# innate2adaptive/decombinator

Hardware: NVIDIA B200
Metric: decombined_reads_per_sec (higher is better)
Workload: dtype u32

## Files before the change

decombinator_b200/csrc/dcb_tables.h:

```cpp
#ifndef DCB_TABLES_H
#define DCB_TABLES_H

#include <stdint.h>

#define DCB_MAX_TAG_LEN 32
#define DCB_MAX_TAGS 255
#define DCB_MAX_READ_LEN 4096
#define DCB_HASH_EMPTY 0xFFFFFFFFu

struct DcbKw {
    uint32_t bits_lo, bits_hi;
    uint8_t len;
    uint8_t first_tag;
    uint8_t n_tags;
    uint8_t tags_off;
    uint32_t pad;
};

struct DcbKwSet {
    int32_t n_kw;
    int32_t kq;
    int32_t bitmap_off;
    int32_t hash_off;
    int32_t hash_mask;
    int32_t kw_off;
    int32_t taglist_off;
    int32_t min_len, max_len;
    int32_t set_id;
};

#define DCB_TAG_WORDS 12
struct DcbTag {
    uint32_t bits_lo, bits_hi;
    uint32_t mask_lo, mask_hi;
    uint32_t edge_lo, edge_hi;
    int16_t jump;
    int16_t region_len;
    uint8_t len;
    uint8_t edge_ok;
    uint8_t next_same_prefix;
    uint8_t pad8;
    int32_t region_off;
    uint32_t pad[3];
};

struct DcbGene {
    int32_t n_tags, split, is_v;
    int32_t tag_off;
    DcbKwSet full, half1, half2;
    int32_t lmin;
    int32_t n_words;
};

struct DcbSeedIndex {
    int32_t q, stride;
    int32_t max_off;
    int32_t wlead;
    int32_t lmin;
    int32_t wbits;
    uint32_t bmul;
    int32_t k, span;
    int32_t ck_off;
    uint32_t c1, c2;
    int32_t cshift;
    int32_t tk_off;
    uint32_t t1;
    int32_t tshift;
    int32_t utag_off;
    int32_t n_v, n_tags;
    int32_t chain_off;
    int32_t head_words;
    int32_t bloom_off;
    int32_t n_words;
    int32_t legacy_words;
    int32_t qq, qstride;
    int32_t fbits;
    uint32_t fmul;
    uint32_t m1, m2;
    int32_t b1, b2;
    int32_t qtab_off;
    int32_t qtab_words;
    int32_t bfilter_off;
    int32_t tq_off, tq_bits;
    uint32_t ta, tb;
    int32_t qwlead;
};
#define DCB_TQ_MORE (1u << 24)
#define DCB_TQ_META(prefix_hi, ctag, len, more) ((uint32_t)(prefix_hi) | ((uint32_t)(ctag) << 16) | ((more) ? DCB_TQ_MORE : 0u) | ((uint32_t)(len) << 25))
#define DCB_TQ_LEN(meta) ((meta) >> 25)
#if defined(__CUDA_ARCH__)
#define DCB_TQ_CTAG(meta) __byte_perm((meta), 0u, 0x4442)
#else
#define DCB_TQ_CTAG(meta) (((meta) >> 16) & 0xFFu)
#endif
#define DCB_TQ_HIBITS(lmin) (2 * (lmin) - 32)
#define DCB_TQ_CMPMASK(lmin) ((2u << DCB_TQ_HIBITS(lmin)) - 1u)
#define DCB_TQ_FREE(lmin) DCB_TQ_META(1u << DCB_TQ_HIBITS(lmin), 0xFF, 127, 0)
#ifndef DCB_FBITS
#define DCB_FBITS 16
#endif
#define DCB_FSLOT(key, fmul, fbits) (((uint32_t)(key) * (fmul)) >> (32 - (fbits)))
#define DCB_QQ(lmin, q) (((lmin) >= 20 && (lmin) <= 22) ? (lmin) - 7 : (q))

#define DCB_CK_FPMASK 0xFFFFF000u
#define DCB_CK_OFFMASK(e) ((e) & 0xFFFu)

struct alignas(16) DcbUTag {
    uint32_t bits_lo, bits_hi;
    uint32_t mask_lo;
    uint32_t mask_hi_len;
};
#define DCB_FAST_MAX_TAG_LEN 28
#define DCB_WBITS_UNION 12
#define DCB_WBITS_SINGLE 11
#define DCB_BLOOM_COPIES 8

#define DCB_IDX_MAXOFF(lmin, q) (((lmin) - (q)) < 11 ? ((lmin) - (q)) : 11)
#define DCB_IDX_STRIDE(lmin, q) (DCB_IDX_MAXOFF(lmin, q) + 1)
#define DCB_IDX_WLEAD(lmin, q) (DCB_IDX_MAXOFF(lmin, q) + 1)
#define DCB_IDX_SPAN(lmin, q) ((DCB_IDX_MAXOFF(lmin, q) + 2) / 2)
#define DCB_IDX_K0(lmin, q) (((lmin) - DCB_IDX_SPAN(lmin, q) + 1) < 15 ? ((lmin) - DCB_IDX_SPAN(lmin, q) + 1) : 15)
#define DCB_IDX_K(lmin, q) ((DCB_IDX_WLEAD(lmin, q) + DCB_IDX_K0(lmin, q)) > 32 ? (32 - DCB_IDX_WLEAD(lmin, q)) : DCB_IDX_K0(lmin, q))

#define DCB_BLOOM_MUL(q) ((0x2C1B3C6Du | 1u) << (32 - 2 * (q)))
#define DCB_BLOOM_BIT(key) (31u - ((key) & 31u))
#define DCB_BLOOM_WORD(win, bmul, wbits) (((uint32_t)(win) * (bmul)) >> (32 - (wbits)))

struct DcbSuffixFilter {
    int32_t kq, fbits;
    uint32_t fmul;
    int32_t n_words;
};
#define DCB_SFILTER_HEAD 4
#define DCB_SFSLOT(key, fmul, fbits) (((uint32_t)(key) * (fmul)) >> (32 - (fbits)))

struct alignas(16) DcbHalfKw {
    uint32_t bits_lo, bits_hi;
    uint8_t len, first_len, n_tags, set;
    uint16_t tags_off, pad;
};
struct DcbHalfIndex {
    int32_t q, stride, kmin;
    int32_t n_v, n_tags;
    int32_t v_split, j_split;
    int32_t t_off;
    int32_t h_off, hshift;
    uint32_t c1, c2;
    int32_t ids_off;
    int32_t kw_off, n_kw;
    int32_t tags_off;
    int32_t n_words;
    int32_t j_ok;
    int32_t j_short;
    int32_t jt_off;
};
#define DCB_HALF_JQ 6
#define DCB_HALF_Q 7
#define DCB_HALF_STRIDE 4
#define DCB_HALF_FREE 0xFFFFFFFFu

#if defined(__CUDACC__)
#define DCB_HD __host__ __device__ __forceinline__
#else
#define DCB_HD inline
#endif

DCB_HD uint32_t dcb_fold64(uint32_t lo, uint32_t hi) {
    uint32_t k = lo * 0x9E3779B1u + hi * 0x85EBCA77u;
    return k ^ (k >> 13);
}
DCB_HD uint32_t dcb_hash32(uint32_t k) {
    k *= 0x9E3779B1u;
    return k ^ (k >> 15);
}

#endif
```

decombinator_b200/csrc/dcr_core.cuh:

```cuda
#ifndef DCR_CORE_CUH
#define DCR_CORE_CUH

#include "dcb_tables.h"
#include "../../include/dcb.h"

#if defined(__CUDA_ARCH__)
#define DCB_COUNT(C, id) atomicAdd(&(C)[id], 1u)
#define DCB_POPC(x) __popc(x)
#define DCB_FUNNEL_R(lo, hi, sh) __funnelshift_r((lo), (hi), (sh))
#define DCB_BREV(x) __brev(x)
#define DCB_CLZ(x) __clz(x)
#define DCB_FFS(x) __ffs(x)
#else
#define DCB_COUNT(C, id) ((C)[id] += 1u)
#define DCB_POPC(x) __builtin_popcount(x)
static inline uint32_t dcb_funnel_r_host(uint32_t lo, uint32_t hi, int sh) {
    sh &= 31;
    return sh ? (lo >> sh) | (hi << (32 - sh)) : lo;
}
static inline uint32_t dcb_brev_host(uint32_t x) {
    x = ((x >> 1) & 0x55555555u) | ((x & 0x55555555u) << 1);
    x = ((x >> 2) & 0x33333333u) | ((x & 0x33333333u) << 2);
    x = ((x >> 4) & 0x0F0F0F0Fu) | ((x & 0x0F0F0F0Fu) << 4);
    x = ((x >> 8) & 0x00FF00FFu) | ((x & 0x00FF00FFu) << 8);
// ... 513 lines not shown
    return v;
}
DCB_HD const DcbTag* gene_tags(const uint32_t* core) {
    return core ? reinterpret_cast<const DcbTag*>(core + reinterpret_cast<const DcbGene*>(core)->tag_off) : nullptr;
}

DCB_HD uint32_t fast_class_lookup(const SeedIdxView& ix, uint32_t wlo, uint32_t whi) {
    uint32_t offs = 0;
    const uint32_t kmask = mask2(ix.k);
#if defined(__CUDA_ARCH__)
#pragma unroll
#endif
    for (int c = 0; c < 2; c++) {
        const int sh = 2 * (ix.wlead - c * ix.span);
        const uint32_t x = ((uint32_t)c << 30) | (DCB_FUNNEL_R(wlo, whi, sh) & kmask);
        const uint32_t p1 = x * ix.c1, p2 = x * ix.c2;
        const uint32_t e1 = ix.ck[p1 >> ix.cshift], e2 = ix.ck[p2 >> ix.cshift];
        offs |= (((e1 ^ p2) & DCB_CK_FPMASK) == 0 ? e1 : 0u) | (((e2 ^ p1) & DCB_CK_FPMASK) == 0 ? e2 : 0u);
    }
    return DCB_CK_OFFMASK(offs);
}

DCB_HD void fast_check_offset(const ReadView& r, const SeedIdxView& ix, int p, int o, uint32_t wlo, uint32_t whi,
                              FullHit& vh, FullHit& jh) {
    const int P = p - o;
    const int sh = 2 * (ix.wlead - o);
    const uint32_t lo = DCB_FUNNEL_R(wlo, whi, sh), hi = whi >> sh;
    const uint32_t f = dcb_fold64(lo & mask2(ix.lmin), ix.lmin > 16 ? (hi & mask2(ix.lmin - 16)) : 0u);
    uint32_t ctag = ix.tk[(f * ix.t1) >> ix.tshift];
    if (P < 0) return;
    while (ctag != 0x1FFu) {
        const DcbUTag u = ix.utag[ctag];
        const int L = (int)(u.mask_hi_len >> 24);
        if (P + L <= r.n) {
            uint32_t tlo = lo, thi = hi;
            if (ix.wlead - o + L > 32) rd_win32(r, P, tlo, thi);
            if (!(((tlo ^ u.bits_lo) & u.mask_lo) | ((thi ^ u.bits_hi) & (u.mask_hi_len & 0x00FFFFFFu)))) {
                if ((int)ctag >= ix.n_v) fullhit_add(jh, (int)ctag - ix.n_v, P);
                else fullhit_add(vh, (int)ctag, P);
            }
        }
        ctag = ix.chain ? ix.chain[ctag] : 0x1FFu;
    }
}

struct alignas(16) DcbTagFin {
    uint32_t edge_lo, edge_hi;
    int16_t jump, region_len;
    uint8_t len, edge_ok, next_same_prefix, pad8;
};
DCB_HD DcbTagFin tag_fin(const DcbTag* tags, int k) {
    return *reinterpret_cast<const DcbTagFin*>(reinterpret_cast<const uint32_t*>(tags + k) + 4);
}

template <bool PADDED>
DCB_HD void rd_win32x(const ReadView& r, int p, uint32_t& lo, uint32_t& hi) {
    if (PADDED) {
        const uint32_t* c0 = r.w + (p >> 4) * r.stride;
        const uint32_t a = c0[0], b = c0[r.stride], c = c0[2 * r.stride];
        const int sh = (p & 15) * 2;
        lo = DCB_FUNNEL_R(a, b, sh);
        hi = DCB_FUNNEL_R(b, c, sh);
    } else {
        rd_win32(r, p, lo, hi);
    }
}

template <bool PADDED>
DCB_HD int fast_v_deletions(const ReadView& r, const DcbTagFin& t, int temp_end_v, int& end_v, int& dels, const ReadView* ri = nullptr) {
    const int f0 = temp_end_v + 1;
    if (!t.edge_ok || f0 >= r.n || f0 < 32) return 0;
    uint32_t lo, hi, rl, rh;
    rd_win32x<PADDED>(r, f0 - 32, lo, hi);
    lo ^= t.edge_lo; hi ^= t.edge_hi;
    if (ri) { uint32_t ilo, ihi; rd_win32x<PADDED>(*ri, f0 - 32, ilo, ihi); lo |= ilo; hi |= ihi; }
    run10(lo, hi, rl, rh);
    rh &= (1u << 14) - 1u;
    if (!(rl | rh)) return 0;
    const int top = rh ? 63 - DCB_CLZ(rh) : 31 - DCB_CLZ(rl);
    dels = 22 - (top >> 1);
    end_v = temp_end_v - dels;
    return 1;
}

template <bool PADDED>
DCB_HD int fast_j_deletions(const ReadView& r, const DcbTagFin& t, int temp_start_j, int end_of_v, int& start_j, int& dels,
                            const ReadView* ri = nullptr) {
    if (!t.edge_ok || temp_start_j < 0) return 0;
    if (PADDED && temp_start_j >= 16 * (r.nw - 1)) return 0;
    int pos0 = end_of_v - temp_start_j;
    if (pos0 < 0) pos0 = 0;
    int imax = r.n - 10 - temp_start_j;
    if (pos0 > 22 || imax < 0) return 0;
    if (imax > 22) imax = 22;
    uint32_t lo, hi, rl, rh;
    rd_win32x<PADDED>(r, temp_start_j, lo, hi);
    lo ^= t.edge_lo; hi ^= t.edge_hi;
    if (ri) { uint32_t ilo, ihi; rd_win32x<PADDED>(*ri, temp_start_j, ilo, ihi); lo |= ilo; hi |= ihi; }
    run10(lo, hi, rl, rh);
    uint64_t r10 = ((uint64_t)rh << 32) | rl;
    r10 &= ~((1ull << (2 * pos0)) - 1);
    r10 &= (1ull << (2 * imax + 2)) - 1;
    if (!r10) return 0;
    const int low = (uint32_t)r10 ? DCB_FFS((uint32_t)r10) - 1 : 32 + DCB_FFS((uint32_t)(r10 >> 32)) - 1;
    dels = low >> 1;
    start_j = temp_start_j + dels;
    return 1;
}

DCB_HD void fast_find(const ReadView& r, const uint32_t* ib, FullHit& vh, FullHit& jh, bool stop_at_two_v) {
    const SeedIdxView ix = seed_idx_view(ib);
    const int last = r.n - ix.q;
    for (int base = 0; base <= last; base += 32 * ix.stride) {
        uint32_t hits = 0;
        for (int i = 0; i < 32; i++) {
            const int p = base + i * ix.stride;
            if (p > last) break;
            const uint32_t win = rd_win16(r, p);
            const uint32_t word = ix.bloom[DCB_BLOOM_WORD(win, ix.bmul, ix.wbits)];
            hits |= ((word >> DCB_BLOOM_BIT(win)) & 1u) << i;
        }
        while (hits) {
            const int i = DCB_FFS(hits) - 1;
            hits &= hits - 1;
            const int p = base + i * ix.stride;
            uint32_t wlo, whi;
            rd_win32(r, p - ix.wlead, wlo, whi);
            for (uint32_t offs = fast_class_lookup(ix, wlo, whi); offs; offs &= offs - 1)
                fast_check_offset(r, ix, p, DCB_FFS(offs) - 1, wlo, whi, vh, jh);
            if (stop_at_two_v && vh.count >= 2) return;
        }
    }
}

#define DCB_HIT_ONE 0x80000000u
#define DCB_HIT_MULTI 0xFFFFFFFFu
#define DCB_HIT_UNKNOWN 0xFFFFFFFEu
DCB_HD uint32_t hit_merge(uint32_t cur, uint32_t c) {
    return cur == 0u ? c : ((c == 0u || c == cur) ? cur : DCB_HIT_MULTI);
}
DCB_HD FullHit hit_decode(uint32_t h) {
    FullHit fh;
    fh.count = h == 0u ? 0 : (h == DCB_HIT_MULTI ? 2 : 1);
    fh.code = h & 0x7FFFFFFFu;
    return fh;
}

DCB_HD uint32_t half_word_of(const FullHit& fh) {
    return fh.count == 0 ? 0u : (fh.count > 1 ? DCB_HIT_MULTI : (DCB_HIT_ONE | fh.code));
}

struct alignas(8) DcbTq { uint32_t x, y; };
struct QIdxView {
    const uint16_t* disp;
    const uint16_t* offs;
    const DcbTq* tq;
    const DcbUTag* utag;
    const uint16_t* chain;
    uint32_t m1, m2, ta, tb, mask2;
    int s1, s2, tqshift;
    int q, stride, lmin, wlead, n_v;
};
DCB_HD QIdxView q_idx_view(const uint32_t* ib, const uint32_t* qtab) {
    const DcbSeedIndex& ix = *reinterpret_cast<const DcbSeedIndex*>(ib);
    QIdxView v;
    v.disp = reinterpret_cast<const uint16_t*>(qtab);
    v.offs = v.disp + ((size_t)1 << ix.b1);
    v.tq = reinterpret_cast<const DcbTq*>(qtab + (ix.tq_off - ix.qtab_off));
    v.utag = reinterpret_cast<const DcbUTag*>(ib + ix.utag_off);
    v.chain = ix.chain_off ? reinterpret_cast<const uint16_t*>(ib + ix.chain_off) : nullptr;
    v.m1 = ix.m1; v.m2 = ix.m2; v.ta = ix.ta; v.tb = ix.tb; v.mask2 = (1u << ix.b2) - 1u;
    v.s1 = 32 - ix.b1; v.s2 = 32 - ix.b2; v.tqshift = 32 - ix.tq_bits;
    v.q = ix.qq; v.stride = ix.qstride; v.lmin = ix.lmin; v.wlead = ix.qwlead; v.n_v = ix.n_v;
    return v;
}
DCB_HD uint32_t q_offsets(const QIdxView& ix, uint32_t x) {
    const uint32_t d = ix.disp[(x * ix.m1) >> ix.s1];
    return ix.offs[(((x * ix.m2) >> ix.s2) + d) & ix.mask2];
}
template <bool PADDED, class Sink>
DCB_HD void q_check_offset(const ReadView& r, const QIdxView& ix, int p, int o, uint32_t wlo, uint32_t whi, Sink& sink) {
    const int P = p - o;
    const int sh = 2 * (ix.wlead - o);
    const uint32_t lo = DCB_FUNNEL_R(wlo, whi, sh), hi = whi >> sh;
    const uint32_t hp = hi & ((1u << DCB_TQ_HIBITS(ix.lmin)) - 1u);
    const DcbTq e = ix.tq[(lo * ix.ta + hp * ix.tb) >> ix.tqshift];
    if (e.x != lo || ((hp ^ e.y) & DCB_TQ_CMPMASK(ix.lmin)) != 0u || P < 0) return;
    uint32_t ctag = DCB_TQ_CTAG(e.y);
    if (!(e.y & DCB_TQ_MORE)) {
        if (P + (int)DCB_TQ_LEN(e.y) <= r.n) sink(ctag, P);
        return;
    }
    while (ctag != 0x1FFu) {
        const DcbUTag u = ix.utag[ctag];
        const int L = (int)(u.mask_hi_len >> 24);
        if (P + L <= r.n) {
            uint32_t tlo = lo, thi = hi;
            if (ix.wlead - o + L > 32) rd_win32x<PADDED>(r, P, tlo, thi);
            if (!(((tlo ^ u.bits_lo) & u.mask_lo) | ((thi ^ u.bits_hi) & (u.mask_hi_len & 0x00FFFFFFu)))) sink(ctag, P);
        }
        ctag = ix.chain ? ix.chain[ctag] : 0x1FFu;
    }
}
struct HitWords {
    uint32_t v, j;
    int n_v;
    DCB_HD void operator()(uint32_t ctag, int P) {
        const bool is_j = (int)ctag >= n_v;
        const uint32_t c = DCB_HIT_ONE | (ctag << 16) | (uint32_t)P;
        const uint32_t m = hit_merge(is_j ? j : v, c);
        v = is_j ? v : m;
        j = is_j ? m : j;
    }
    DCB_HD void decode(FullHit& vh, FullHit& jh) const {
        vh = hit_decode(v);
        jh = hit_decode(j);
        jh.code -= (uint32_t)n_v << 16;
    }
};
struct ExcProbe {
    uint32_t p01, p23;
    uint32_t e0;
    bool over;
};
DCB_HD ExcProbe exc_probe_none() {
    ExcProbe x;
    x.p01 = x.p23 = 0xFFFFFFFFu; x.e0 = 0; x.over = false;
    return x;
}
DCB_HD void exc_probe_add(ExcProbe& x, int slot, uint32_t pos) {
    const uint32_t sh = (slot & 1) * 16, m = 0xFFFFu << sh;
    uint32_t& w = slot < 2 ? x.p01 : x.p23;
    w = (w & ~m) | (pos << sh);
}
DCB_HD ExcProbe exc_probe_load(const uint32_t* read, const uint16_t* pos, const uint8_t* kind, const uint32_t* index, uint32_t ri) {
    ExcProbe x = exc_probe_none();
    uint32_t e = index[ri >> 5];
    while (read[e] < ri) e++;
    x.e0 = e;
    int n = 0;
    for (; read[e] == ri; e++) {
        if (kind[e] == 3) continue;
        if (n < 4) exc_probe_add(x, n, pos[e]);
        n++;
    }
    x.over = n > 4;
    return x;
}
DCB_HD bool exc_in_span(const ExcProbe& x, int lo, int hi) {
    const int a = (int)(x.p01 & 0xFFFFu), b = (int)(x.p01 >> 16), c = (int)(x.p23 & 0xFFFFu), d = (int)(x.p23 >> 16);
    return (a >= lo && a < hi) || (b >= lo && b < hi) || (c >= lo && c < hi) || (d >= lo && d < hi);
}
struct HitWordsX {
    HitWords hw;
    const ExcProbe* xp;
    const DcbUTag* utag;
    DCB_HD bool fake(uint32_t c) const {
        const int P = (int)(c & 0xFFFFu);
        return exc_in_span(*xp, P, P + (int)(utag[(c >> 16) & 0x7FFFu].mask_hi_len >> 24));
    }
    DCB_HD void operator()(uint32_t ctag, int P) {
        if (xp) {
            const uint32_t c = DCB_HIT_ONE | (ctag << 16) | (uint32_t)P;
            uint32_t& cur = (int)ctag >= hw.n_v ? hw.j : hw.v;
            if (cur != 0u && cur != c && cur != DCB_HIT_MULTI) {
                if (fake(c)) return;
                if (fake(cur)) { cur = c; return; }
            }
        }
        hw(ctag, P);
    }
    DCB_HD void finish() {
        if (!xp) return;
        if (hw.v != 0u && hw.v != DCB_HIT_MULTI && fake(hw.v)) hw.v = 0u;
        if (hw.j != 0u && hw.j != DCB_HIT_MULTI && fake(hw.j)) hw.j = 0u;
    }
};
DCB_HD void q_find(const ReadView& r, const uint32_t* ib, FullHit& vh, FullHit& jh, const ExcProbe* xp = nullptr) {
    const DcbSeedIndex& hd = *reinterpret_cast<const DcbSeedIndex*>(ib);
    const QIdxView ix = q_idx_view(ib, ib + hd.qtab_off);
    const uint8_t* filt = reinterpret_cast<const uint8_t*>(ib + hd.bfilter_off);
    HitWordsX hw;
    hw.hw.v = 0; hw.hw.j = 0; hw.hw.n_v = ix.n_v; hw.xp = xp; hw.utag = ix.utag;
    for (int p = 0; p + ix.q <= r.n; p += ix.stride) {
        const uint32_t win = rd_win16(r, p);
        if (!filt[DCB_FSLOT(win, hd.fmul, hd.fbits)]) continue;
        uint32_t wlo, whi;
        rd_win32(r, p - ix.wlead, wlo, whi);
        for (uint32_t offs = q_offsets(ix, DCB_FUNNEL_R(wlo, whi, 2 * ix.wlead)); offs; offs &= offs - 1)
            q_check_offset<false>(r, ix, p, DCB_FFS(offs) - 1, wlo, whi, hw);
    }
    hw.finish();
    hw.hw.decode(vh, jh);
}

enum { FAST_DONE = 0, FAST_DEFER = 1 };

template <bool PADDED>
DCB_HD int dcr_fast_from_hits(const ReadView& r, const DcbTag* vtags, const DcbTag* jtags, const FullHit& vh,
                              const FullHit& jh, const DcrParams& prm, int both_frames, dcb_result& out,
                              dcb_cnt_t* C, const bool use_xp = false, const ExcProbe xp = exc_probe_none()) {
    if (vh.count == 0) return FAST_DEFER;
    if (vh.count > 1) {
        if (both_frames) return FAST_DEFER;
        DCB_COUNT(C, DCB_C_multiple_v_matches);
        return FAST_DONE;
    }
    const DcbTagFin vt = tag_fin(vtags, fullhit_tag(vh));
    VJ v, j;
    v.idx = fullhit_tag(vh); v.seqpos = fullhit_pos(vh);
    if (!fast_v_deletions<PADDED>(r, vt, v.seqpos + vt.jump - 1, v.pos, v.dels)) return FAST_DEFER;
    if (use_xp) {
        const int f0 = v.seqpos + vt.jump;
        if (exc_in_span(xp, f0 - 32, f0)) return FAST_DEFER;
    }
    if (jh.count == 0) return FAST_DEFER;
    if (jh.count > 1) {
        if (both_frames) return FAST_DEFER;
        DCB_COUNT(C, DCB_C_multiple_j_matches);
        DCB_COUNT(C, DCB_C_VJ_assignment_failed);
        return FAST_DONE;
    }
    const DcbTagFin jt = tag_fin(jtags, fullhit_tag(jh));
    j.idx = fullhit_tag(jh); j.seqpos = fullhit_pos(jh) + (int)jt.len;
    if (!fast_j_deletions<PADDED>(r, jt, fullhit_pos(jh) - jt.jump, v.pos + 1, j.pos, j.dels)) return FAST_DEFER;
    if (use_xp) {
        const int f0 = v.seqpos + vt.jump, tsj = fullhit_pos(jh) - jt.jump;
        const int lo = v.seqpos < f0 - 32 ? v.seqpos : f0 - 32;
        int hi = j.seqpos > tsj + 32 ? j.seqpos : tsj + 32;
        if (f0 > hi) hi = f0;
        if (exc_in_span(xp, lo, hi)) return FAST_DEFER;
// ... 453 lines not shown
```

decombinator_b200/csrc/tagset.cpp:

```cpp
#include "dcb_internal.h"

#include <algorithm>
#include <cstring>
#include <map>
#include <string>
#include <vector>

namespace {

inline int base_code(char c) {
    switch (c) {
        case 'A': return 0; case 'C': return 1; case 'G': return 2; case 'T': return 3;
        default: return -1;
    }
}

bool pack64(const std::string& s, size_t from, size_t n, uint32_t& lo, uint32_t& hi) {
    uint64_t v = 0;
    lo = hi = 0;
    for (size_t i = 0; i < n; i++) {
        int c = base_code(s[from + i]);
        if (c < 0) return false;
        v |= (uint64_t)c << (2 * i);
    }
    lo = (uint32_t)v; hi = (uint32_t)(v >> 32);
    return true;
}

uint32_t pow2_at_least(uint32_t x) {
    uint32_t p = 16;
    while (p < x) p <<= 1;
    return p;
}

struct Blob {
    std::vector<uint32_t> w;
    int32_t reserve(size_t n_words) {
        int32_t off = (int32_t)w.size();
        w.resize(w.size() + n_words, 0u);
        return off;
    }
    void align4() { while (w.size() % 4) w.push_back(0u); }
};

struct Cuckoo {
    uint32_t c1 = 1, c2 = 1;
    int bits = 4;
    std::vector<uint32_t> key, val;
    std::vector<uint8_t> used;
    uint32_t h(uint32_t k, int which) const { return (k * (which ? c2 : c1)) >> (32 - bits); }
    bool build(const std::vector<std::pair<uint32_t, uint32_t>>& items, int bits_, uint32_t c1_, uint32_t c2_) {
        bits = bits_; c1 = c1_ | 1u; c2 = c2_ | 1u;
        const size_t n = (size_t)1 << bits;
        key.assign(n, 0); val.assign(n, 0); used.assign(n, 0);
        for (auto it : items) {
            uint32_t k = it.first, v = it.second;
            int which = 0;
            bool placed = false;
            for (int kick = 0; kick < 500; kick++) {
                uint32_t s = h(k, which);
                if (!used[s]) { used[s] = 1; key[s] = k; val[s] = v; placed = true; break; }
                uint32_t s2 = h(k, which ^ 1);
                if (!used[s2]) { used[s2] = 1; key[s2] = k; val[s2] = v; placed = true; break; }
                std::swap(k, key[s]); std::swap(v, val[s]);
                which = (h(k, 0) == s) ? 1 : 0;
            }
            if (!placed) return false;
        }
        return true;
    }
};

bool build_cuckoo(Cuckoo& ck, const std::vector<std::pair<uint32_t, uint32_t>>& items) {
    int bits = 4;
    while (((size_t)1 << bits) < 2 * items.size() + 2) bits++;
    uint64_t rng = 0x2545F4914F6CDD1Dull;
    for (int grow = 0; grow < 6; grow++, bits++) {
        for (int attempt = 0; attempt < 64; attempt++) {
            rng ^= rng << 13; rng ^= rng >> 7; rng ^= rng << 17;
            if (ck.build(items, bits, (uint32_t)rng, (uint32_t)(rng >> 32))) return true;
        }
    }
    return false;
}

void build_kwset(Blob& b, DcbKwSet& ks, const std::vector<std::string>& list) {
    std::vector<std::string> kws;
    std::vector<std::vector<int>> members;
    std::map<std::string, int> seen;
    for (size_t i = 0; i < list.size(); i++) {
        if (list[i].empty()) continue;
        auto it = seen.find(list[i]);
        if (it == seen.end()) {
            seen[list[i]] = (int)kws.size();
            kws.push_back(list[i]);
            members.push_back({(int)i});
        } else {
            members[it->second].push_back((int)i);
        }
    }
    int min_len = 1 << 30, max_len = 0;
    for (auto& k : kws) { min_len = std::min(min_len, (int)k.size()); max_len = std::max(max_len, (int)k.size()); }
    if (kws.empty()) { min_len = 1; max_len = 1; }
    ks.n_kw = (int)kws.size();
    ks.min_len = min_len; ks.max_len = max_len;
    ks.kq = std::min(min_len, 6);
    struct Ent { uint32_t key; int len; int id; };
    std::vector<Ent> ents;
    for (size_t i = 0; i < kws.size(); i++) {
        uint32_t lo, hi;
        pack64(kws[i], kws[i].size() - ks.kq, ks.kq, lo, hi);
        ents.push_back({lo, (int)kws[i].size(), (int)i});
    }
    std::stable_sort(ents.begin(), ents.end(), [](const Ent& a, const Ent& c) {
        if (a.key != c.key) return a.key < c.key;
        return a.len > c.len;
    });
    size_t bitmap_words = ((size_t)1 << (2 * ks.kq)) / 32;
    if (bitmap_words == 0) bitmap_words = 1;
    ks.bitmap_off = b.reserve(bitmap_words);
    size_t n_groups = 0;
    for (size_t i = 0; i < ents.size(); i++) if (i == 0 || ents[i].key != ents[i - 1].key) n_groups++;
    uint32_t hsize = pow2_at_least((uint32_t)(2 * n_groups + 1));
    ks.hash_mask = (int32_t)(hsize - 1);
    ks.hash_off = b.reserve(hsize);
    for (uint32_t i = 0; i < hsize; i++) b.w[ks.hash_off + i] = DCB_HASH_EMPTY;
    ks.kw_off = b.reserve(4 * ents.size());
    size_t total_tags = 0;
    for (auto& m : members) total_tags += m.size();
    ks.taglist_off = b.reserve((total_tags + 3) / 4 + 1);
    uint8_t* taglist = reinterpret_cast<uint8_t*>(&b.w[ks.taglist_off]);
    size_t tl = 0;
    for (size_t i = 0; i < ents.size(); i++) {
        const std::string& s = kws[ents[i].id];
        DcbKw kw;
        std::memset(&kw, 0, sizeof(kw));
        pack64(s, 0, s.size(), kw.bits_lo, kw.bits_hi);
        kw.len = (uint8_t)s.size();
        kw.first_tag = (uint8_t)members[ents[i].id][0];
        kw.n_tags = (uint8_t)members[ents[i].id].size();
        kw.tags_off = (uint8_t)tl;
        for (int t : members[ents[i].id]) taglist[tl++] = (uint8_t)t;
        std::memcpy(&b.w[ks.kw_off + 4 * i], &kw, sizeof(kw));
        b.w[ks.bitmap_off + (ents[i].key >> 5)] |= 1u << (ents[i].key & 31);
        if (i == 0 || ents[i].key != ents[i - 1].key) {
            size_t cnt = 1;
            while (i + cnt < ents.size() && ents[i + cnt].key == ents[i].key) cnt++;
            uint32_t h = dcb_hash32(ents[i].key) & (hsize - 1);
            while (b.w[ks.hash_off + h] != DCB_HASH_EMPTY) h = (h + 1) & (hsize - 1);
            b.w[ks.hash_off + h] = (ents[i].key << 16) | ((uint32_t)i << 8) | (uint32_t)cnt;
        }
    }
}

struct Chd {
    uint32_t m1 = 1, m2 = 1;
    int b1 = 1, b2 = 1;
    std::vector<uint16_t> disp, slot;
    bool build(const std::vector<std::pair<uint32_t, uint32_t>>& items, int b1_, int b2_, uint32_t m1_, uint32_t m2_) {
        b1 = b1_; b2 = b2_; m1 = m1_; m2 = m2_;
        const size_t n1 = (size_t)1 << b1, n2 = (size_t)1 << b2;
        std::vector<std::vector<size_t>> bucket(n1);
        for (size_t i = 0; i < items.size(); i++) bucket[(items[i].first * m1) >> (32 - b1)].push_back(i);
        std::vector<size_t> order(n1);
        for (size_t i = 0; i < n1; i++) order[i] = i;
        std::stable_sort(order.begin(), order.end(), [&](size_t a, size_t c) { return bucket[a].size() > bucket[c].size(); });
        disp.assign(n1, 0); slot.assign(n2, 0);
        std::vector<uint8_t> used(n2, 0);
        std::vector<uint32_t> base, at;
        for (size_t bi : order) {
            const auto& bk = bucket[bi];
            if (bk.empty()) break;
            base.clear();
            for (size_t i : bk) base.push_back((items[i].first * m2) >> (32 - b2));
            for (size_t i = 0; i < base.size(); i++)
                for (size_t k = i + 1; k < base.size(); k++)
                    if (base[i] == base[k]) return false;
            bool placed = false;
            for (uint32_t d = 0; d < n2 && d < 65536u && !placed; d++) {
                bool ok = true;
                for (uint32_t x : base) if (used[(x + d) & (n2 - 1)]) { ok = false; break; }
                if (!ok) continue;
                for (size_t i = 0; i < bk.size(); i++) {
                    const uint32_t s = (base[i] + d) & (uint32_t)(n2 - 1);
                    used[s] = 1; slot[s] = (uint16_t)items[bk[i]].second;
                }
                disp[bi] = (uint16_t)d;
                placed = true;
            }
            if (!placed) return false;
        }
        return true;
    }
};

bool build_chd(Chd& chd, const std::vector<std::pair<uint32_t, uint32_t>>& items, int q) {
    if (2 * q > 30) return false;
    int b2 = 4;
    while (((size_t)1 << b2) < 2 * items.size() + 2) b2++;
    int b1 = b2 > 4 ? b2 - 3 : 1;
    if (b2 > 2 * q) return false;
    uint64_t rng = 0xD1B54A32D192ED03ull;
    for (int attempt = 0; attempt < 4096; attempt++) {
        rng ^= rng << 13; rng ^= rng >> 7; rng ^= rng << 17;
        const uint32_t m1 = ((uint32_t)rng | 1u) << (32 - 2 * q), m2 = ((uint32_t)(rng >> 32) | 1u) << (32 - 2 * q);
        if (chd.build(items, b1, b2, m1, m2)) return true;
    }
    return false;
}

int seed_q(int lmin) { return lmin >= 18 ? 9 : lmin >= 12 ? 8 : lmin >= 8 ? 6 : lmin; }

}

bool dcb_build_seed_index(const std::vector<std::string>* gene_v, const std::vector<std::string>* gene_j, int lmin,
                          int wbits, std::vector<uint32_t>& out) {
    Blob b;
    DcbSeedIndex idx;
    std::memset(&idx, 0, sizeof(idx));
    b.reserve((sizeof(DcbSeedIndex) + 3) / 4);
    b.align4();
    idx.q = seed_q(lmin);
    idx.lmin = lmin;
    idx.max_off = DCB_IDX_MAXOFF(lmin, idx.q);
    idx.stride = DCB_IDX_STRIDE(lmin, idx.q);
    idx.wlead = DCB_IDX_WLEAD(lmin, idx.q);
    idx.wbits = wbits;
    idx.span = DCB_IDX_SPAN(lmin, idx.q);
    idx.k = DCB_IDX_K(lmin, idx.q);
    if (idx.k < 1 || idx.k > 15) return false;
    if (idx.q < 3 || idx.q > 9 || lmin > 32 || wbits < 2 || wbits > 2 * idx.q - 5 || wbits > 27) return false;
    idx.bmul = DCB_BLOOM_MUL(idx.q);

    std::vector<const std::string*> all;
    idx.n_v = gene_v ? (int32_t)gene_v->size() : 0;
    if (gene_v) for (auto& s : *gene_v) all.push_back(&s);
    if (gene_j) for (auto& s : *gene_j) all.push_back(&s);
    idx.n_tags = (int32_t)all.size();
    if (all.empty() || all.size() > 510) return false;

    std::map<uint32_t, uint32_t> seeds;
    std::map<uint32_t, uint32_t> classkeys;
    std::map<std::pair<uint32_t, uint32_t>, int> prefixes;
    std::vector<int> next_same(all.size(), 0x1FF);
    for (size_t t = 0; t < all.size(); t++) {
        const std::string& s = *all[t];
        if ((int)s.size() < lmin || s.size() > DCB_FAST_MAX_TAG_LEN) return false;
        uint32_t lo, hi;
        for (int o = 0; o <= idx.max_off; o++) {
            if (!pack64(s, o, idx.q, lo, hi)) return false;
            seeds[lo] |= 1u << o;
            const int c = o / idx.span;
            pack64(s, o - c * idx.span, idx.k, lo, hi);
            classkeys[((uint32_t)c << 30) | lo] |= 1u << o;
        }
        pack64(s, 0, lmin, lo, hi);
        auto key = std::make_pair(lo, hi);
        auto it = prefixes.find(key);
        if (it == prefixes.end()) prefixes[key] = (int)t;
        else {
            int k = it->second;
            while (next_same[k] != 0x1FF) k = next_same[k];
            next_same[k] = (int)t;
        }
    }
    {
        std::vector<std::pair<uint32_t, uint32_t>> items(classkeys.begin(), classkeys.end());
        Cuckoo ck;
        if (!build_cuckoo(ck, items)) return false;
        idx.c1 = ck.c1; idx.c2 = ck.c2; idx.cshift = 32 - ck.bits;
        const size_t slots = (size_t)1 << ck.bits;
        idx.ck_off = b.reserve(slots);
        for (size_t i = 0; i < slots; i++) {
            if (!ck.used[i]) { b.w[idx.ck_off + i] = 0u; continue; }
            const uint32_t other = ck.h(ck.key[i], 0) == i ? ck.key[i] * ck.c2 : ck.key[i] * ck.c1;
            b.w[idx.ck_off + i] = (other & DCB_CK_FPMASK) | ck.val[i];
        }
    }
    {
        std::vector<std::pair<uint32_t, int>> items;
        for (auto& kv : prefixes) items.emplace_back(dcb_fold64(kv.first.first, kv.first.second), kv.second);
        for (size_t i = 0; i < items.size(); i++)
            for (size_t k = i + 1; k < items.size(); k++)
                if (items[i].first == items[k].first) return false;
        uint64_t rng = 0x9E3779B97F4A7C15ull;
        bool done = false;
        for (int bits = 9; bits <= 14 && !done; bits++) {
            if (((size_t)1 << bits) < 2 * items.size()) continue;
            std::vector<int> slot((size_t)1 << bits);
            for (int attempt = 0; attempt < 20000 && !done; attempt++) {
                rng ^= rng << 13; rng ^= rng >> 7; rng ^= rng << 17;
                const uint32_t m = (uint32_t)rng | 1u;
                std::fill(slot.begin(), slot.end(), -1);
                bool ok = true;
                for (auto& it : items) {
                    int& sl = slot[(it.first * m) >> (32 - bits)];
                    if (sl >= 0) { ok = false; break; }
                    sl = it.second;
                }
                if (!ok) continue;
                idx.t1 = m; idx.tshift = 32 - bits;
                idx.tk_off = b.reserve(((size_t)1 << bits) / 2);
                uint16_t* tk = reinterpret_cast<uint16_t*>(&b.w[idx.tk_off]);
                for (size_t i = 0; i < slot.size(); i++) tk[i] = slot[i] >= 0 ? (uint16_t)slot[i] : (uint16_t)0x1FF;
                done = true;
            }
        }
        if (!done) return false;
    }
    b.align4();
    idx.utag_off = b.reserve(4 * all.size());
    bool any_chain = false;
    for (size_t t = 0; t < all.size(); t++) {
        const std::string& s = *all[t];
        DcbUTag u;
        pack64(s, 0, s.size(), u.bits_lo, u.bits_hi);
        const uint64_t m = (1ull << (2 * s.size())) - 1ull;
        u.mask_lo = (uint32_t)m;
        u.mask_hi_len = (uint32_t)(m >> 32) | ((uint32_t)s.size() << 24);
        std::memcpy(&b.w[idx.utag_off + 4 * t], &u, sizeof(u));
        if (next_same[t] != 0x1FF) any_chain = true;
    }
    idx.chain_off = 0;
    if (any_chain) {
        idx.chain_off = b.reserve((all.size() + 1) / 2);
        uint16_t* ch = reinterpret_cast<uint16_t*>(&b.w[idx.chain_off]);
        for (size_t t = 0; t < all.size(); t++) ch[t] = (uint16_t)next_same[t];
    }
    b.align4();
    idx.head_words = (int32_t)b.w.size();
    const size_t words = (size_t)1 << wbits;
    idx.bloom_off = b.reserve(words);
    for (auto& kv : seeds)
        b.w[idx.bloom_off + DCB_BLOOM_WORD(kv.first, idx.bmul, wbits)] |= 1u << DCB_BLOOM_BIT(kv.first);
    b.align4();
    idx.legacy_words = (int32_t)b.w.size();
    {
        idx.qq = DCB_QQ(lmin, idx.q);
        idx.qstride = lmin - idx.qq + 1;
        if (idx.qstride > 12) { idx.qq = idx.q; idx.qstride = idx.stride; }
        std::map<uint32_t, uint32_t> seeds2;
        for (size_t t = 0; t < all.size(); t++) {
            uint32_t lo, hi;
            for (int o = 0; o < idx.qstride; o++) {
                if (!pack64(*all[t], o, idx.qq, lo, hi)) return false;
                seeds2[lo] |= 1u << o;
            }
        }
        std::vector<std::pair<uint32_t, uint32_t>> items(seeds2.begin(), seeds2.end());
        Chd chd;
        if (!build_chd(chd, items, idx.qq)) return false;
        idx.m1 = chd.m1; idx.m2 = chd.m2; idx.b1 = chd.b1; idx.b2 = chd.b2;
        const size_t n1 = (size_t)1 << chd.b1, n2 = (size_t)1 << chd.b2;
        idx.qtab_off = b.reserve((n1 + n2 + 1) / 2);
        uint16_t* t16 = reinterpret_cast<uint16_t*>(&b.w[idx.qtab_off]);
        for (size_t i = 0; i < n1; i++) t16[i] = chd.disp[i];
        for (size_t i = 0; i < n2; i++) t16[n1 + i] = chd.slot[i];
        b.align4();
        idx.tq_off = 0; idx.tq_bits = 0; idx.ta = idx.tb = 1;
        if (lmin >= 17 && lmin <= 23 && all.size() <= 255) {
            const uint32_t himask = (1u << DCB_TQ_HIBITS(lmin)) - 1u;
            uint64_t rng2 = 0xA0761D6478BD642Full;
            bool done = false;
            for (int bits = 8; bits <= 12 && !done; bits++) {
                if (((size_t)1 << bits) < 4 * prefixes.size()) continue;
                std::vector<int> slot((size_t)1 << bits);
                for (int attempt = 0; attempt < 4000 && !done; attempt++) {
                    rng2 ^= rng2 << 13; rng2 ^= rng2 >> 7; rng2 ^= rng2 << 17;
                    const uint32_t ta = (uint32_t)rng2 | 1u, tb = (uint32_t)(rng2 >> 32) | 1u;
                    std::fill(slot.begin(), slot.end(), -1);
                    bool ok = true;
                    for (auto& kv : prefixes) {
                        int& sl = slot[(kv.first.first * ta + (kv.first.second & himask) * tb) >> (32 - bits)];
                        if (sl >= 0) { ok = false; break; }
                        sl = kv.second;
                    }
                    if (!ok) continue;
                    idx.ta = ta; idx.tb = tb; idx.tq_bits = bits;
                    idx.tq_off = b.reserve((size_t)2 << bits);
                    for (size_t i = 0; i < slot.size(); i++) {
                        uint32_t lo = 0, meta = DCB_TQ_FREE(lmin);
                        if (slot[i] >= 0) {
                            const std::string& t = *all[slot[i]];
                            uint32_t hi;
                            pack64(t, 0, lmin, lo, hi);
                            meta = DCB_TQ_META(hi & himask, slot[i], t.size(), (int)t.size() > lmin || next_same[slot[i]] != 0x1FF);
                        }
                        b.w[idx.tq_off + 2 * i] = lo; b.w[idx.tq_off + 2 * i + 1] = meta;
                    }
                    done = true;
                }
            }
        }
        b.align4();
        idx.qwlead = idx.qstride - 1;
        idx.qtab_words = (int32_t)b.w.size() - idx.qtab_off;
        idx.fbits = DCB_FBITS;
        idx.fmul = DCB_BLOOM_MUL(idx.qq);
        if (idx.fbits > 2 * idx.qq) idx.fbits = 2 * idx.qq;
        idx.bfilter_off = b.reserve(((size_t)1 << idx.fbits) / 4);
        uint8_t* f8 = reinterpret_cast<uint8_t*>(&b.w[idx.bfilter_off]);
        for (auto& kv : seeds2) f8[DCB_FSLOT(kv.first, idx.fmul, idx.fbits)] = 1;
    }
    b.align4();
    idx.n_words = (int32_t)b.w.size();
    std::memcpy(&b.w[0], &idx, sizeof(idx));
    out = std::move(b.w);
    return true;
}

bool dcb_build_half_index(const dcb_tagset* v, const dcb_tagset* j, std::vector<uint32_t>& out) {
    DcbHalfIndex hx;
    std::memset(&hx, 0, sizeof(hx));
    hx.q = DCB_HALF_Q; hx.stride = DCB_HALF_STRIDE; hx.kmin = hx.q + hx.stride - 1;
    hx.n_v = v->n_tags; hx.n_tags = v->n_tags + j->n_tags;
    hx.v_split = v->split; hx.j_split = j->split;
    struct Kw { std::string s; int set; std::vector<int> tags; };
    std::vector<Kw> kws;
    hx.j_ok = 1;
    for (int t = 0; t < j->n_tags; t++)
        if (j->split < hx.kmin || (int)j->tags[t].size() - j->split < hx.kmin) hx.j_ok = 0;
    hx.j_short = hx.j_ok ? 0 : 1;
    for (int t = 0; t < j->n_tags; t++)
        if (j->split < DCB_HALF_JQ || (int)j->tags[t].size() - j->split < DCB_HALF_JQ) hx.j_short = 0;
    for (int gi = 0; gi < 2; gi++) {
        const dcb_tagset* ts = gi ? j : v;
        if (gi == 1 && !hx.j_ok && !hx.j_short) break;
        const int kmin = (gi == 1 && !hx.j_ok) ? DCB_HALF_JQ : hx.kmin;
        for (int half = 0; half < 2; half++) {
            std::map<std::string, size_t> seen;
            for (int t = 0; t < ts->n_tags; t++) {
                const std::string h = half ? ts->tags[t].substr(ts->split) : ts->tags[t].substr(0, ts->split);
                if ((int)h.size() < kmin || h.size() > 31 || ts->tags[t].size() > 31) return false;
                auto it = seen.find(h);
                if (it == seen.end()) { seen[h] = kws.size(); kws.push_back({h, 2 * gi + half, {t}}); }
                else kws[it->second].tags.push_back(t);
            }
        }
    }
    if (kws.empty() || kws.size() > 255) return false;
    Blob b;
    b.reserve((sizeof(DcbHalfIndex) + 3) / 4);
    b.align4();
    hx.t_off = b.reserve(((size_t)1 << (2 * hx.q)) / 2);
    uint16_t* t16 = reinterpret_cast<uint16_t*>(&b.w[hx.t_off]);
    std::map<uint32_t, std::vector<int>> by_prefix;
    std::map<uint32_t, std::vector<int>> by_six;
    std::vector<uint8_t> tag_ids;
    std::vector<DcbHalfKw> recs(kws.size());
    for (size_t i = 0; i < kws.size(); i++) {
        const Kw& k = kws[i];
        uint32_t lo, hi;
        if (k.set >= 2 && hx.j_short) {
            if (!pack64(k.s, 0, DCB_HALF_JQ, lo, hi)) return false;
            by_six[lo].push_back((int)i);
        } else {
            for (int o = 0; o < hx.stride; o++) {
                if (!pack64(k.s, o, hx.q, lo, hi)) return false;
                t16[lo] |= (uint16_t)(1u << (4 * k.set + o));
            }
            pack64(k.s, 0, hx.kmin, lo, hi);
            by_prefix[((uint32_t)k.set << 28) | lo].push_back((int)i);
        }
        if (!pack64(k.s, 0, k.s.size(), lo, hi)) return false;
        DcbHalfKw& r = recs[i];
        std::memset(&r, 0, sizeof(r));
        pack64(k.s, 0, k.s.size(), r.bits_lo, r.bits_hi);
        const dcb_tagset* ts = k.set >= 2 ? j : v;
        r.len = (uint8_t)k.s.size();
        r.first_len = (uint8_t)ts->tags[k.tags[0]].size();
        if (k.tags.size() > 15) return false;
        r.n_tags = (uint8_t)k.tags.size();
        r.set = (uint8_t)k.set;
        if (tag_ids.size() + k.tags.size() > 65535) return false;
        r.tags_off = (uint16_t)tag_ids.size();
        for (int t : k.tags) tag_ids.push_back((uint8_t)t);
    }
    std::vector<uint8_t> ids;
    std::vector<std::pair<uint32_t, uint32_t>> items;
    for (auto& kv : by_prefix) {
        if (kv.second.size() > 255 || ids.size() > 255) return false;
        items.emplace_back(kv.first, (uint32_t)ids.size() | ((uint32_t)kv.second.size() << 8));
        for (int i : kv.second) ids.push_back((uint8_t)i);
    }
    std::vector<uint16_t> jt;
    if (hx.j_short) {
        jt.assign((size_t)1 << (2 * DCB_HALF_JQ), 0);
        for (auto& kv : by_six) {
            if (kv.second.size() > 255 || ids.size() > 255) return false;
            jt[kv.first] = (uint16_t)(ids.size() | (kv.second.size() << 8));
            for (int i : kv.second) ids.push_back((uint8_t)i);
        }
    }
    Cuckoo ck;
    if (!build_cuckoo(ck, items)) return false;
    hx.c1 = ck.c1; hx.c2 = ck.c2; hx.hshift = 32 - ck.bits;
    const size_t slots = (size_t)1 << ck.bits;
    b.align4();
    hx.h_off = b.reserve(2 * slots);
    for (size_t i = 0; i < slots; i++) {
        b.w[hx.h_off + 2 * i] = ck.used[i] ? ck.key[i] : DCB_HALF_FREE;
        b.w[hx.h_off + 2 * i + 1] = ck.used[i] ? ck.val[i] : 0u;
    }
    hx.ids_off = b.reserve((ids.size() + 3) / 4 + 1);
    std::memcpy(&b.w[hx.ids_off], ids.data(), ids.size());
    b.align4();
    hx.n_kw = (int32_t)recs.size();
    hx.kw_off = b.reserve(4 * recs.size());
    std::memcpy(&b.w[hx.kw_off], recs.data(), sizeof(DcbHalfKw) * recs.size());
    hx.tags_off = b.reserve((tag_ids.size() + 3) / 4 + 1);
// ... 159 lines not shown
```

Measured before the change: 24.72 billion.

## Replace CHD perfect hash with two-way cuckoo table for seed offsets

Swaps the two-level CHD perfect-hash lookup (a displacement read followed by a dependent slot read) for a two-choice cuckoo table of key/offset pairs. The two probes are independent and can be issued in parallel, and the stored key allows an exact membership check. The cost is a larger table (8-byte entries instead of 16-bit slots), so more cache or shared memory is used per lookup, and it relies on an existing cuckoo builder succeeding.

```diff
diff --git a/decombinator_b200/csrc/dcb_tables.h b/decombinator_b200/csrc/dcb_tables.h
--- a/decombinator_b200/csrc/dcb_tables.h
+++ b/decombinator_b200/csrc/dcb_tables.h
@@ -85,6 +85,8 @@
     uint32_t ta, tb;
     int32_t qwlead;
 };
+struct alignas(8) DcbOSet { uint32_t key, offs; };
+#define DCB_OSET_FREE 0xFFFFFFFFu
 #define DCB_TQ_MORE (1u << 24)
 #define DCB_TQ_META(prefix_hi, ctag, len, more) ((uint32_t)(prefix_hi) | ((uint32_t)(ctag) << 16) | ((more) ? DCB_TQ_MORE : 0u) | ((uint32_t)(len) << 25))
 #define DCB_TQ_LEN(meta) ((meta) >> 25)
diff --git a/decombinator_b200/csrc/dcr_core.cuh b/decombinator_b200/csrc/dcr_core.cuh
--- a/decombinator_b200/csrc/dcr_core.cuh
+++ b/decombinator_b200/csrc/dcr_core.cuh
@@ -689,31 +689,30 @@
 
 struct alignas(8) DcbTq { uint32_t x, y; };
 struct QIdxView {
-    const uint16_t* disp;
-    const uint16_t* offs;
+    const DcbOSet* oset;
     const DcbTq* tq;
     const DcbUTag* utag;
     const uint16_t* chain;
-    uint32_t m1, m2, ta, tb, mask2;
-    int s1, s2, tqshift;
+    uint32_t m1, m2, ta, tb;
+    int s2, tqshift;
     int q, stride, lmin, wlead, n_v;
 };
 DCB_HD QIdxView q_idx_view(const uint32_t* ib, const uint32_t* qtab) {
     const DcbSeedIndex& ix = *reinterpret_cast<const DcbSeedIndex*>(ib);
     QIdxView v;
-    v.disp = reinterpret_cast<const uint16_t*>(qtab);
-    v.offs = v.disp + ((size_t)1 << ix.b1);
+    v.oset = reinterpret_cast<const DcbOSet*>(qtab);
     v.tq = reinterpret_cast<const DcbTq*>(qtab + (ix.tq_off - ix.qtab_off));
     v.utag = reinterpret_cast<const DcbUTag*>(ib + ix.utag_off);
     v.chain = ix.chain_off ? reinterpret_cast<const uint16_t*>(ib + ix.chain_off) : nullptr;
-    v.m1 = ix.m1; v.m2 = ix.m2; v.ta = ix.ta; v.tb = ix.tb; v.mask2 = (1u << ix.b2) - 1u;
-    v.s1 = 32 - ix.b1; v.s2 = 32 - ix.b2; v.tqshift = 32 - ix.tq_bits;
+    v.m1 = ix.m1; v.m2 = ix.m2; v.ta = ix.ta; v.tb = ix.tb;
+    v.s2 = 32 - ix.b2; v.tqshift = 32 - ix.tq_bits;
     v.q = ix.qq; v.stride = ix.qstride; v.lmin = ix.lmin; v.wlead = ix.qwlead; v.n_v = ix.n_v;
     return v;
 }
-DCB_HD uint32_t q_offsets(const QIdxView& ix, uint32_t x) {
-    const uint32_t d = ix.disp[(x * ix.m1) >> ix.s1];
-    return ix.offs[(((x * ix.m2) >> ix.s2) + d) & ix.mask2];
+DCB_HD uint32_t q_offsets(const QIdxView& ix, uint32_t w) {
+    const uint32_t x = w & ((1u << (2 * ix.q)) - 1u);
+    const DcbOSet e1 = ix.oset[(w * ix.m1) >> ix.s2], e2 = ix.oset[(w * ix.m2) >> ix.s2];
+    return (e1.key == x ? e1.offs : 0u) | (e2.key == x ? e2.offs : 0u);
 }
 template <bool PADDED, class Sink>
 DCB_HD void q_check_offset(const ReadView& r, const QIdxView& ix, int p, int o, uint32_t wlo, uint32_t whi, Sink& sink) {
diff --git a/decombinator_b200/csrc/tagset.cpp b/decombinator_b200/csrc/tagset.cpp
--- a/decombinator_b200/csrc/tagset.cpp
+++ b/decombinator_b200/csrc/tagset.cpp
@@ -153,62 +153,6 @@
     }
 }
 
-struct Chd {
-    uint32_t m1 = 1, m2 = 1;
-    int b1 = 1, b2 = 1;
-    std::vector<uint16_t> disp, slot;
-    bool build(const std::vector<std::pair<uint32_t, uint32_t>>& items, int b1_, int b2_, uint32_t m1_, uint32_t m2_) {
-        b1 = b1_; b2 = b2_; m1 = m1_; m2 = m2_;
-        const size_t n1 = (size_t)1 << b1, n2 = (size_t)1 << b2;
-        std::vector<std::vector<size_t>> bucket(n1);
-        for (size_t i = 0; i < items.size(); i++) bucket[(items[i].first * m1) >> (32 - b1)].push_back(i);
-        std::vector<size_t> order(n1);
-        for (size_t i = 0; i < n1; i++) order[i] = i;
-        std::stable_sort(order.begin(), order.end(), [&](size_t a, size_t c) { return bucket[a].size() > bucket[c].size(); });
-        disp.assign(n1, 0); slot.assign(n2, 0);
-        std::vector<uint8_t> used(n2, 0);
-        std::vector<uint32_t> base, at;
-        for (size_t bi : order) {
-            const auto& bk = bucket[bi];
-            if (bk.empty()) break;
-            base.clear();
-            for (size_t i : bk) base.push_back((items[i].first * m2) >> (32 - b2));
-            for (size_t i = 0; i < base.size(); i++)
-                for (size_t k = i + 1; k < base.size(); k++)
-                    if (base[i] == base[k]) return false;
-            bool placed = false;
-            for (uint32_t d = 0; d < n2 && d < 65536u && !placed; d++) {
-                bool ok = true;
-                for (uint32_t x : base) if (used[(x + d) & (n2 - 1)]) { ok = false; break; }
-                if (!ok) continue;
-                for (size_t i = 0; i < bk.size(); i++) {
-                    const uint32_t s = (base[i] + d) & (uint32_t)(n2 - 1);
-                    used[s] = 1; slot[s] = (uint16_t)items[bk[i]].second;
-                }
-                disp[bi] = (uint16_t)d;
-                placed = true;
-            }
-            if (!placed) return false;
-        }
-        return true;
-    }
-};
-
-bool build_chd(Chd& chd, const std::vector<std::pair<uint32_t, uint32_t>>& items, int q) {
-    if (2 * q > 30) return false;
-    int b2 = 4;
-    while (((size_t)1 << b2) < 2 * items.size() + 2) b2++;
-    int b1 = b2 > 4 ? b2 - 3 : 1;
-    if (b2 > 2 * q) return false;
-    uint64_t rng = 0xD1B54A32D192ED03ull;
-    for (int attempt = 0; attempt < 4096; attempt++) {
-        rng ^= rng << 13; rng ^= rng >> 7; rng ^= rng << 17;
-        const uint32_t m1 = ((uint32_t)rng | 1u) << (32 - 2 * q), m2 = ((uint32_t)(rng >> 32) | 1u) << (32 - 2 * q);
-        if (chd.build(items, b1, b2, m1, m2)) return true;
-    }
-    return false;
-}
-
 int seed_q(int lmin) { return lmin >= 18 ? 9 : lmin >= 12 ? 8 : lmin >= 8 ? 6 : lmin; }
 
 }
@@ -347,15 +291,20 @@
                 seeds2[lo] |= 1u << o;
             }
         }
-        std::vector<std::pair<uint32_t, uint32_t>> items(seeds2.begin(), seeds2.end());
-        Chd chd;
-        if (!build_chd(chd, items, idx.qq)) return false;
-        idx.m1 = chd.m1; idx.m2 = chd.m2; idx.b1 = chd.b1; idx.b2 = chd.b2;
-        const size_t n1 = (size_t)1 << chd.b1, n2 = (size_t)1 << chd.b2;
-        idx.qtab_off = b.reserve((n1 + n2 + 1) / 2);
-        uint16_t* t16 = reinterpret_cast<uint16_t*>(&b.w[idx.qtab_off]);
-        for (size_t i = 0; i < n1; i++) t16[i] = chd.disp[i];
-        for (size_t i = 0; i < n2; i++) t16[n1 + i] = chd.slot[i];
+        if (2 * idx.qq > 30) return false;
+        const int ks = 32 - 2 * idx.qq;
+        std::vector<std::pair<uint32_t, uint32_t>> items;
+        for (auto& kv : seeds2) items.emplace_back(kv.first << ks, kv.second);
+        Cuckoo ck;
+        if (!build_cuckoo(ck, items)) return false;
+        idx.m1 = ck.c1 << ks; idx.m2 = ck.c2 << ks; idx.b1 = 0; idx.b2 = ck.bits;
+        const size_t n2 = (size_t)1 << ck.bits;
+        idx.qtab_off = b.reserve(2 * n2);
+        DcbOSet* os = reinterpret_cast<DcbOSet*>(&b.w[idx.qtab_off]);
+        for (size_t i = 0; i < n2; i++) {
+            os[i].key = ck.used[i] ? ck.key[i] >> ks : DCB_OSET_FREE;
+            os[i].offs = ck.used[i] ? ck.val[i] : 0u;
+        }
         b.align4();
         idx.tq_off = 0; idx.tq_bits = 0; idx.ta = idx.tb = 1;
         if (lmin >= 17 && lmin <= 23 && all.size() <= 255) {
```

Measured after the change: 23.95 billion (median of 6 runs). 0.969x the previous value.
